# okieraised/rs-face-detection-tflite

Measured on AMD Instinct MI355X. Metric: faces/sec at batch=256 (256x256 back-camera) per GPU, higher is better.
Workload: dtype f32

## Files before the change

rs-face-detection-tflite_amd/csrc/engine.cpp:

```cpp
#include "engine.hpp"
#include "launch.hpp"

#include <mutex>

#include <algorithm>
#include <cstdio>
#include <cstdlib>
#include <cstring>
#include <functional>
#include <stdexcept>

namespace mi {

void hip_check(hipError_t e, const char* what) {
    if (e != hipSuccess) throw std::runtime_error(std::string(what) + ": " + hipGetErrorString(e));
}

namespace {
constexpr int kHeadStreams = 4;

void same_pad(int in, int k, int stride, int out, int* before) {
    int total = std::max(0, (out - 1) * stride + k - in);
    *before = total / 2;
}
// ... 34 lines not shown
}

void Model::invalidate_graphs() {
    if (!graphs_.empty()) (void)hipDeviceSynchronize();
    for (auto& kv : graphs_) hipGraphExecDestroy(kv.second);
    graphs_.clear();
}

void Model::set_option(const std::string& key, int value) {
    if (key == "chunk") chunk_ = std::max(0, value);
    else if (key == "graph") use_graph_ = value != 0;
    else if (key == "fuse") { fuse_level_ = std::min(5, std::max(0, value)); dirty_ = true; }
    else if (key == "res_budget") { res_budget_ = std::min(156, std::max(16, value)) * 1024; dirty_ = true; }
    else if (key == "pipe") { pipe_max_ = std::min(4, std::max(0, value)); dirty_ = true; }
    else if (key == "small_chain") { small_chain_ = std::max(0, std::min(value, 64)); if (d_small_) { hipFree(d_small_); d_small_ = nullptr; small_floats_ = 0; } invalidate_graphs(); }
    else if (key == "pipe_rows") { pipe_rows_ = (value == 1 || value == 2 || value == 4) ? value : 0; }
    else if (key == "pipe_band") { pipe_band_ = std::max(0, std::min(value, 4096)); }
    else if (key == "strip") { strip_ = value != 0; }
    else if (key == "stem_fuse") { stem_fuse_ = value != 0; }
    else if (key == "stem_mfma") { stem_mfma_ = value != 0; }
    else if (key == "pair_fuse") { pair_fuse_ = value != 0; }
    else if (key == "mdb_band") { mdb_band_ = std::max(0, std::min(value, 4096)); }
    else if (key == "mchain") { mchain_ = value != 0; }
    else if (key == "tail") { tail_ = value != 0; dirty_ = true; }
    else if (key == "tail_pre") { tail_pre_ = std::max(0, std::min(value, 2)); }
    else if (key == "tail_g") { tail_g_ = std::max(0, std::min(value, 64)); }
    else if (key == "band") { band_ = std::max(0, std::min(value, 2)); dirty_ = true; }
    else if (key == "band_test_fail") { band_test_fail_ = value != 0; }
    else if (key == "band_test_absent") { band_test_absent_ = std::max(0, std::min(value, 256)); }
    else if (key == "band_test_gen") { band_gen_ = static_cast<unsigned>(std::max(0, value)); band_gen_force_ = true; }
    else if (key == "band_wide") { band_wide_ok_ = value != 0; dirty_ = true; }
    else if (key == "band_fork") { band_fork_ = value != 0; dirty_ = true; }
    else if (key == "band_nw") { band_nw_ = std::max(8, std::min(value, 256)); dirty_ = true; }
    else if (key == "fork") { fork_ = value != 0; }
    else if (key == "heads") { head_streams_opt_ = std::min(kHeadStreams, std::max(1, value)); dirty_ = true; }
    else if (key == "reuse") { reuse_ = value != 0; dirty_ = true; }
    else if (key == "lanes") lanes_ = std::min(4, std::max(1, value));
    else throw std::runtime_error("unknown option '" + key + "'");
    invalidate_graphs();
    chunk_cap_ = 0;
}

int Model::get_option(const std::string& key) const {
    if (key == "chunk") return chunk_;
    if (key == "graph") return use_graph_;
    if (key == "fuse") return fuse_level_;
    if (key == "res_budget") return res_budget_ / 1024;
    if (key == "pipe") return pipe_max_;
    if (key == "small_chain") return small_chain_;
    if (key == "pipe_rows") return pipe_rows_;
    if (key == "pipe_band") return pipe_band_;
    if (key == "strip") return strip_;
    if (key == "stem_fuse") return stem_fuse_;
    if (key == "stem_mfma") return stem_mfma_;
    if (key == "pair_fuse") return pair_fuse_;
    if (key == "mdb_band") return mdb_band_;
    if (key == "mchain") return mchain_;
    if (key == "tail") return tail_;
    if (key == "tail_pre") return tail_pre_;
    if (key == "tail_g") return tail_g_;
    if (key == "band") return band_;
    if (key == "band_fork") return band_fork_;
    if (key == "band_wide") return band_wide_ok_;
    if (key == "band_nw") return band_nw_;
    if (key == "band_fail_streak") return band_fail_streak_;
    if (key == "band_wraps") return band_wraps_;
    if (key == "fork") return fork_;
    if (key == "heads") return head_streams_opt_;
    if (key == "reuse") return reuse_;
    if (key == "lanes") return lanes_;
    throw std::runtime_error("unknown option '" + key + "'");
}

void Model::rebuild() {
    if (d_small_) { hipFree(d_small_); d_small_ = nullptr; small_floats_ = 0; }
    hip_check(hipSetDevice(device_), "hipSetDevice");
    invalidate_graphs();
    plan_ = build_plan(parse_tflite(blob_.data(), blob_.size()), fuse_level_, pipe_max_, res_budget_, tail_ != 0);
    const Graph& g = plan_.graph;
    if (!reuse_) {
// ... 1366 lines not shown
    return stats;
}

void Model::enqueue_chunk(const float* in, int chunk_start, int F, hipStream_t s, std::vector<hipEvent_t>* marks,
                          std::vector<std::string>* labels) {
    const Graph& g = plan_.graph;
    auto mark = [&] {
        if (!marks) return;
        hipEvent_t ev;
        hip_check(hipEventCreate(&ev), "hipEventCreate");
        hip_check(hipEventRecord(ev, s), "hipEventRecord");
        marks->push_back(ev);
    };
    mark();
    const bool fork = fork_ && !marks && lanes_ == 1;
    hipStream_t const trunk = s;
    unsigned used_heads = 0;
    auto node_event = [&](size_t k) {
        if (head_events_.size() < plan_.nodes.size() + 2 + kHeadStreams) head_events_.resize(plan_.nodes.size() + 2 + kHeadStreams, nullptr);
        if (!head_events_[k]) hip_check(hipEventCreateWithFlags(&head_events_[k], hipEventDisableTiming), "hipEventCreate");
        return head_events_[k];
    };
    int fused_behind = 0;
    const bool band = band_use_ && chunk_start == 0;
    for (size_t i = 0; i < plan_.nodes.size(); i++) {
        const Node& n = plan_.nodes[i];
        if (n.kind == Node::Reshape || n.kind == Node::Concat) continue;
        if (band && static_cast<int>(i) >= band_first_ && !band_node_runs_[i]) {
            if (static_cast<int>(i) > band_first_) {
                if (labels) labels->push_back("(inside the band launch)");
                mark();
                continue;
            }
            if (labels) labels->push_back("bandnet_kernel");
            BandLaunch a;
            a.prog = d_band_prog_; a.nstages = band_nstages_; a.NW = band_nw_used_; a.F = F; a.lds_bytes = band_lds_bytes_;
            a.tiles_floats = band_tiles_floats_;
            a.dw_floats = band_dw_floats_; a.ws_frame_floats = band_ws_frame_floats_;
            long fs = 0;
            a.base[0] = d_band_ws_;
            a.base[1] = const_cast<float*>(tensor_ptr(band_stem_out_, in, chunk_start, &fs));
            a.cv2 = band_cv2_ ? 1 : 0;
            a.xb = band_xb_ ? 1 : 0;
            a.wide = band_wide_ ? 1 : 0;
            for (size_t k = 0; k < band_ext_.size(); k++) {
                long efs = 0;
                a.base[2 + k] = band_ext_[k].out_k >= 0 ? d_out_[static_cast<size_t>(band_ext_[k].out_k)] : tensor_ptr_mut(band_ext_[k].tensor, chunk_start, &efs);
            }
            a.consts = d_band_consts_; a.sync = d_band_sync_; a.fail = d_band_fail_;
            a.absent_mod = band_test_absent_;
            int rc = 0;
            for (int rep_ = 0; rep_ < (marks ? profile_inner_ : 1) && rc == 0; rep_++) rc = launch_bandnet(a, trunk);
            if (rc != 0) throw std::runtime_error(std::string("kernel launch failed: ") + hipGetErrorString(static_cast<hipError_t>(rc)));
            for (size_t j = i; fork && j < plan_.nodes.size(); j++)
                if (!band_node_runs_[j] && event_after_[j]) hip_check(record_event(node_event(j), trunk), "hipEventRecord");
            mark();
            continue;
        }
        if (fused_behind > 0) {
            fused_behind--;
            if (labels) labels->push_back("(fused into previous launch)");
            if (fork && event_after_[i]) hip_check(record_event(node_event(i), trunk), "hipEventRecord");
            mark();
            continue;
        }
        s = trunk;
        const bool in_line = band && n.gemm_head && head_wait_[i] >= 0 && !band_node_runs_[static_cast<size_t>(head_wait_[i])];
        if (fork && head_slot_[i] >= 0 && !in_line) {
            while (static_cast<int>(head_streams_.size()) <= head_slot_[i]) {
                hipStream_t st;
                hip_check(hipStreamCreateWithFlags(&st, hipStreamNonBlocking), "hipStreamCreate");
                head_streams_.push_back(st);
            }
            s = head_streams_[head_slot_[i]];
            if (head_wait_[i] >= 0) {
                hip_check(wait_event(s, node_event(static_cast<size_t>(head_wait_[i]))), "hipStreamWaitEvent");
            } else {
                hip_check(record_event(node_event(plan_.nodes.size()), trunk), "hipEventRecord");
                hip_check(wait_event(s, node_event(plan_.nodes.size())), "hipStreamWaitEvent");
            }
            used_heads |= 1u << head_slot_[i];
        }
        const auto& si = g.tensors[n.in[0]].shape;
// ... 31 lines not shown
                    break;
                }
                if (strip_ && stem_fuse_ && node_stem_[i] >= 0 && !u8_.frames) {
                    const size_t j = i + 1;
                    if (node_mwalk_[j] >= 0 && !event_after_[i] && head_slot_[j] < 0) {
                        const Node& c = plan_.nodes[j];
                        const auto& co = g.tensors[c.out].shape;
                        DblockArgs d;
                        long ofs = 0;
                        d.out = tensor_ptr_mut(c.out, chunk_start, &ofs); d.out_fs = ofs;
                        d.B = F; d.H = so[1]; d.W = so[2]; d.C = so[3]; d.Cm = g.tensors[c.members[0].out].shape[3]; d.Co = co[3];
                        d.hi1 = c.members[0].act == ACT_RELU6 ? 6.f : INFINITY;
                        d.hi2 = c.members[1].act == ACT_RELU6 ? 6.f : INFINITY;
                        d.skip1 = 1; d.skip2_from_a = 1;
                        d.act1 = c.members[0].act; d.act2 = c.members[1].act;
                        d.mconsts = d_weights_ + node_mwalk_[j];
                        d.stem_in = ip; d.stem_in_fs = in_fs; d.stem_consts = d_weights_ + node_stem_[i];
                        d.stem_hi = n.act == ACT_RELU6 ? 6.f : INFINITY;
                        d.band_rows = mdb_band_;
                        if (mdblock_kernel_supports(d)) {
                            if (labels) labels->back() = "mdblock_kernel<stem+pair>";
                            rc = launch_mdblock(d, s);
                            fused_behind = 1;
                            break;
                        }
                    }
                }
                ConvArgs a;
                a.in = ip; a.out = op; a.in_fs = in_fs; a.out_fs = out_fs;
                a.w = d_weights_ + node_w_[i];
                a.B = F; a.H = si[1]; a.W = si[2]; a.C = si[3]; a.Ho = so[1]; a.Wo = so[2]; a.Co = so[3]; a.Cop = (a.Co + 3) & ~3;
                a.KH = n.KH; a.KW = n.KW; a.sh = n.sh; a.sw = n.sw;
                if (n.padding == Padding::Same) { same_pad(a.H, a.KH, a.sh, a.Ho, &a.pt); same_pad(a.W, a.KW, a.sw, a.Wo, &a.pl); }
                if (n.ept >= 0) { a.pt = n.ept; a.pl = n.epl; }
                a.ep = ep;
                a.no_mfma = stem_mfma_ ? 0 : 1;
                if (u8_.frames && plan_.storage[n.in[0]].root == plan_.storage[g.inputs[0]].root) {
                    if (!conv_takes_u8(a)) throw std::runtime_error("plan: this graph's first convolution has no u8 input form");
                    a.in_u8 = u8_.frames + static_cast<long>(chunk_start) * u8_.frame_bytes;
                    a.u8_lut = u8_.lut; a.u8_frame_bytes = u8_.frame_bytes; a.u8_row_bytes = u8_.row_bytes;
                }
                if (labels) labels->back() = conv_kernel_label(a);
                rc = launch_conv(a, s);
                break;
            }
            case Node::Dw: {
// ... 258 lines not shown
                if (a.has_dw && n.ept >= 0) { a.pt = n.ept; a.pl = n.epl; }
                a.ep = ep;
                a.w_strip = node_strip_[i] >= 0 ? d_weights_ + node_strip_[i] : nullptr;
                a.w_mwalk = node_mwalk_[i] >= 0 ? d_weights_ + node_mwalk_[i] : nullptr;
                if (strip_ && pair_fuse_ && node_pair_[i] >= 0 && i + 1 < plan_.nodes.size() && !event_after_[i] && head_slot_[i + 1] < 0 && head_slot_[i] < 0) {
                    const Node& nb = plan_.nodes[i + 1];
                    {
                        DblockArgs d;
                        long ofs = 0;
                        d.in = ip; d.in_fs = in_fs;
                        d.out = tensor_ptr_mut(nb.out, chunk_start, &ofs); d.out_fs = ofs;
                        d.B = F; d.H = si[1]; d.W = si[2]; d.C = si[3]; d.Cm = si[3]; d.Co = si[3];
                        d.hi1 = n.act == ACT_RELU6 ? 6.f : INFINITY;
                        d.hi2 = nb.act == ACT_RELU6 ? 6.f : INFINITY;
                        d.skip1 = 1; d.skip2_from_a = 1;
                        d.act1 = n.act; d.act2 = nb.act;
                        d.mconsts = d_weights_ + node_pair_[i];
                        d.band_rows = mdb_band_;
                        const bool apart = d.out + d.out_fs * F <= d.in || d.in + d.in_fs * F <= d.out;
                        if (apart && mdblock_kernel_supports(d)) {
                            if (labels) labels->back() = "mdblock_kernel<pair>";
                            rc = launch_mdblock(d, s);
                            fused_behind = 1;
                            break;
                        }
                    }
                }
                if (strip_ && ms2_kernel_supports(a)) {
                    if (labels) { char buf[96]; labels->back() = ms2_kernel_label(a, buf, sizeof buf); }
                    rc = launch_ms2(a, s);
                    break;
                }
                if (strip_ && mwalk_kernel_supports(a)) {
                    if (labels) { char buf[96]; labels->back() = mwalk_kernel_label(a, buf, sizeof buf); }
                    rc = launch_mwalk(a, s);
                    break;
                }
                const bool strip = strip_ && strip_kernel_supports(a);
                const bool mstrip = strip_ && !strip && mstrip_kernel_supports(a);
                if (mstrip && mchain_ && lanes_ == 1) {
                    std::vector<BlockArgs> run{a};
                    for (size_t j = i + 1; j < plan_.nodes.size() && run.size() < 8; j++) {
                        const Node& m = plan_.nodes[j];
                        if (m.kind != Node::Block || m.w < 0 || m.in.size() != 1 || m.in[0] != plan_.nodes[j - 1].out || node_strip_[j] < 0 || head_slot_[j] >= 0) break;
                        const auto& mi_ = g.tensors[m.in[0]].shape;
                        const auto& mo_ = g.tensors[m.out].shape;
// ... 3 lines not shown
                        bb.out = tensor_ptr_mut(m.out, chunk_start, &bb.out_fs);
                        bb.has_dw = 1;
                        bb.w_dw = d_weights_ + node_w_[j];
                        bb.b_dw = node_b_[j] >= 0 ? d_weights_ + node_b_[j] : nullptr;
                        bb.w_pw = d_weights_ + node_w2_[j];
                        bb.w_strip = d_weights_ + node_strip_[j];
                        bb.B = F; bb.H = mi_[1]; bb.W = mi_[2]; bb.C = mi_[3]; bb.Ho = mo_[1]; bb.Wo = mo_[2]; bb.Co = mo_[3];
                        bb.sh = m.sh; bb.sw = m.sw;
                        if (m.padding == Padding::Same) { same_pad(bb.H, 3, bb.sh, bb.Ho, &bb.pt); same_pad(bb.W, 3, bb.sw, bb.Wo, &bb.pl); }
                        if (m.ept >= 0) break;
                        bb.ep.bias = node_b2_[j] >= 0 ? d_weights_ + node_b2_[j] : nullptr;
                        bb.ep.alpha = node_alpha_[j] >= 0 ? d_weights_ + node_alpha_[j] : nullptr;
                        bb.ep.act = m.act;
                        if (m.res >= 0) {
                            if (m.res != m.in[0] || m.res_mode != RES_DIRECT || m.res_after) break;
                            bb.ep.res = bb.in; bb.ep.res_fs = bb.in_fs; bb.ep.res_mode = RES_DIRECT; bb.ep.res_C = bb.C;
                            bb.ep.res_H = bb.H; bb.ep.res_W = bb.W;
                        }
                        run.push_back(bb);
                        if (!mstrip_chain_supports(run.data(), static_cast<int>(run.size()))) { run.pop_back(); break; }
                    }
                    if (run.size() >= 2) {
                        if (labels) { char buf[96]; snprintf(buf, sizeof buf, "mstrip_chain_kernel<%d,%d>", a.C / 4, a.ep.act == ACT_RELU ? 1 : 0); labels->back() = buf; }
                        rc = launch_mstrip_chain(run.data(), static_cast<int>(run.size()), s);
                        fused_behind = static_cast<int>(run.size()) - 1;
                        break;
                    }
                }
                if (labels) { char buf[96]; labels->back() = strip ? strip_kernel_label(a, buf, sizeof buf) : (mstrip ? mstrip_kernel_label(a, buf, sizeof buf) : block_kernel_label(a, buf, sizeof buf)); }
                rc = strip ? launch_strip(a, s) : (mstrip ? launch_mstrip(a, s) : launch_block(a, s));
                break;
            }
            default: {
                EltArgs a;
                a.a = ip; a.a_fs = in_fs; a.out = op; a.out_fs = out_fs; a.alpha = ep.alpha; a.act = n.act;
                a.B = F; a.H = dim(si, 1); a.W = dim(si, 2); a.C = si.back();
                a.Ho = dim(so, 1); a.Wo = dim(so, 2); a.Co = so.back();
                if (si.size() != 4) { a.H = 1; a.W = 1; a.C = static_cast<int>(g.tensors[n.in[0]].elems()); a.Ho = a.Wo = 1; a.Co = a.C; }
                if (n.kind == Node::Add) {
                    a.b = tensor_ptr(n.in[1], in, chunk_start, &a.b_fs);
                    rc = launch_add(a, s);
                } else if (n.kind == Node::Act) {
                    rc = launch_act(a, s);
                } else if (n.kind == Node::MaxPool) {
                    a.p0 = n.filter_h; a.p1 = n.filter_w; a.p2 = n.sh; a.p3 = n.sw;
                    rc = launch_maxpool(a, s);
                } else if (n.kind == Node::Pad) {
                    const auto& pv = g.tensors[n.pads].i32;
// ... 221 lines not shown
            d_in_stage_ = nullptr;
            hip_check(hipMalloc(reinterpret_cast<void**>(&d_in_stage_), need * sizeof(float)), "hipMalloc stage");
            in_stage_floats_ = need;
        }
        hip_check(hipMemcpyAsync(d_in_stage_, in, need * sizeof(float), hipMemcpyHostToDevice, s), "H2D input");
        din = d_in_stage_;
    }
    run_device(din, batch, s);
    for (int k = 0; k < num_outputs(); k++) {
        if (!outs[k]) continue;
        hip_check(hipMemcpyAsync(outs[k], d_out_[k], output_elems(k) * sizeof(float) * batch,
                                 mem == 0 ? hipMemcpyDeviceToHost : hipMemcpyDeviceToDevice, s), "copy outputs");
    }
    if (mem == 0 || !stream) hip_check(hipStreamSynchronize(s), "hipStreamSynchronize");
}

size_t Model::debug_tensor(int tensor, int frame, float* dst, size_t cap) {
    const Graph& g = plan_.graph;
    if (tensor < 0 || tensor >= static_cast<int>(g.tensors.size())) throw std::runtime_error("tensor index out of range");
    if (frame < 0 || frame >= last_chunk_frames_) throw std::runtime_error("frame outside the last chunk");
    const Storage& st = plan_.storage[tensor];
    bool produced = false;
    for (const Node& n : plan_.nodes) produced |= (n.out == tensor);
    if (!produced) throw std::runtime_error("tensor was fused away (or is an input/constant)");
    long fs;
    float* p = tensor_ptr_mut(tensor, 0, &fs);
    size_t n = std::min(cap, g.tensors[tensor].elems());
    hip_check(hipDeviceSynchronize(), "sync");
    hip_check(hipMemcpy(dst, p + static_cast<long>(frame) * fs, n * sizeof(float), hipMemcpyDeviceToHost), "D2H debug");
    (void)st;
    return n;
}

}
```

rs-face-detection-tflite_amd/csrc/engine.hpp:

```cpp
#pragma once

#include <hip/hip_runtime.h>

#include <map>
#include <memory>
#include <string>
#include <vector>

#include "plan.hpp"

namespace mi {

void hip_check(hipError_t e, const char* what);

class Model {
   public:
    Model(const uint8_t* bytes, size_t n, int device);
    ~Model();
    Model(const Model&) = delete;
    Model& operator=(const Model&) = delete;

    int device() const { return device_; }
    const Graph& graph() const { return plan_.graph; }
    const Plan& plan() const { return plan_; }
// ... 47 lines not shown
    std::vector<hipEvent_t> lane_events_;
    std::vector<int> head_slot_;
    std::vector<int> head_wait_;
    std::vector<char> event_after_;
    std::vector<hipStream_t> head_streams_;
    std::vector<hipEvent_t> head_events_;
    bool dirty_ = true;

    float* d_weights_ = nullptr;
    std::vector<long> node_w_, node_b_, node_w2_, node_b2_, node_alpha_;
    std::vector<long> node_pair_;
    std::vector<long> node_stem_;
    std::vector<long> node_mwalk_;
    std::vector<long> node_strip_;
    struct MemberOff { long w = -1, b = -1, w2 = -1, b2 = -1, alpha = -1, strip = -1; };
    int profile_inner_ = 1;
    std::vector<std::vector<MemberOff>> chain_off_;
    std::vector<std::vector<MemberOff>> chain_head_off_;

    ResStage* d_programs_ = nullptr;
    TailStage* d_tail_programs_ = nullptr;
    std::vector<std::vector<long>> tail_wa_, tail_wc_;
    int mchain_ = 1;
    int tail_ = 1;
    int tail_pre_ = 0;
    int tail_g_ = 0;
    std::vector<std::vector<long>> res_wblk_;
    std::vector<std::vector<long>> res_cblob_;
    std::vector<long> node_prog_;
    float* d_arena_ = nullptr;
    size_t arena_floats_ = 0;
    int chunk_cap_ = 0;
    int batch_cap_ = 0;
    std::vector<float*> d_out_;
    float* d_in_stage_ = nullptr;
    size_t in_stage_floats_ = 0;
    int last_chunk_frames_ = 0;

    int band_ = 1;
    int band_nw_ = 128;
    int band_nw_used_ = 0;
    bool band_ready_ = false;
    bool band_use_ = false;
    bool band_ran_ = false;
    bool band_test_fail_ = false;
    int band_test_absent_ = 0;
    int band_fail_streak_ = 0;
    bool band_disabled_ = false;
    unsigned band_gen_ = 0;
    bool band_gen_force_ = false;
    int band_wraps_ = 0;
    size_t band_ws_bytes_ = 0;
    int band_first_ = 0;
    int band_stem_out_ = -1;
    int band_nstages_ = 0, band_lds_bytes_ = 0, band_max_frames_ = 0, band_dw_floats_ = 0;
    int band_tiles_floats_ = 0;
    long band_ws_frame_floats_ = 0;
    struct BandExt { int out_k = -1, tensor = -1; };
    std::vector<BandExt> band_ext_;
    std::vector<char> band_node_runs_;
// ... 38 lines not shown
```

rs-face-detection-tflite_amd/csrc/kernels.hpp:

```cpp
#pragma once

#include <cstddef>
#include <cstdint>

namespace mi {

enum ActKind : int { ACT_NONE = 0, ACT_RELU = 1, ACT_RELU6 = 2, ACT_PRELU = 3 };
enum ResMode : int { RES_NONE = 0, RES_DIRECT = 1, RES_MAXPOOL = 2, RES_UP2X = 3 };

struct Epilogue {
    const float* bias = nullptr;
    const float* alpha = nullptr;
    const float* res = nullptr;
    long res_fs = 0;
    int res_mode = RES_NONE;
    int res_C = 0;
    int res_W = 0, res_H = 0;
    int act = ACT_NONE;
    int res_after = 0;
};

struct ConvArgs {
    const float* in = nullptr;
    const uint8_t* in_u8 = nullptr;
// ... 238 lines not shown
bool strip_shape_ok(int C, int Co);
int strip_consts_floats(int C);
void strip_pack_consts(int C, const float* w_dw, const float* b_dw, const float* w_pw, const float* bias, const float* alpha, int act, float* dst);
const char* strip_kernel_label(const BlockArgs& a, char* buf, size_t cap);
int launch_mwalk(const BlockArgs& a, void* stream);
bool mwalk_kernel_supports(const BlockArgs& a);
bool mwalk_shape_ok(int W, int C, int Co);
int mwalk_consts_floats(int W, int C, int Co);
void mwalk_pack_consts(int W, int C, int Co, const float* w_dw, const float* b_dw, const float* w_pw, const float* bias, const float* alpha, int act, float* dst);
const char* mwalk_kernel_label(const BlockArgs& a, char* buf, size_t cap);
int launch_ms2(const BlockArgs& a, void* stream);
bool ms2_kernel_supports(const BlockArgs& a);
bool ms2_shape_ok(int W, int C, int Co, bool skip);
int ms2_consts_floats(int W, int C, int Co, bool skip);
void ms2_pack_consts(int W, int C, int Co, bool skip, const float* w_dw, const float* b_dw, const float* w_pw, const float* bias, const float* alpha, int act, float* dst);
const char* ms2_kernel_label(const BlockArgs& a, char* buf, size_t cap);
int launch_mstrip(const BlockArgs& a, void* stream);
bool mstrip_kernel_supports(const BlockArgs& a);
bool mstrip_shape_ok(int C, int Co);
int mstrip_consts_floats(int C);
void mstrip_pack_consts(int C, const float* w_dw, const float* b_dw, const float* w_pw, const float* bias, const float* alpha, int act, float* dst);
const char* mstrip_kernel_label(const BlockArgs& a, char* buf, size_t cap);
bool mstrip_chain_supports(const BlockArgs* blocks, int n);
int launch_mstrip_chain(const BlockArgs* blocks, int n, void* stream);
bool strip_pipe_supports(const BlockArgs* blocks, int n);
bool strip_pipe_shape_ok(int C, int W);
bool strip_tail_shape_ok(int C, int Co, int H, int W);
int strip_consts_s2_floats(int C, int Co);
void strip_pack_consts_s2(int C, int Co, const float* w_dw, const float* b_dw, const float* w_pw, const float* bias, const float* alpha, int act, float* dst);
int launch_strip_pipe(const BlockArgs* blocks, int n, void* stream);
const char* strip_pipe_label(const BlockArgs* blocks, int n, char* buf, size_t cap);
int strip_pipe_rows_per_step(int H, int hint = 0);
int launch_chain(const ChainArgs& a, void* stream);

struct BneckBlock {
    const float* w1 = nullptr;
    const float* w2 = nullptr;
    const float* consts = nullptr;
    float hi1 = 0.f, hi2 = 0.f;
    const float* mconsts = nullptr;
    int act1 = ACT_RELU, act2 = ACT_RELU;
};
constexpr int kMaxBneck = 6;
struct BneckArgs {
    const float* in = nullptr;
    float* out = nullptr;
    long in_fs = 0, out_fs = 0;
// ... 154 lines not shown
```

rs-face-detection-tflite_amd/csrc/mstrip_kernels.hip:

```cpp
#include <hip/hip_runtime.h>

#include <algorithm>
#include <cstdint>
#include <cstdio>
#include <cstdlib>
#include <type_traits>
#include <utility>

#include "kernels.hpp"
#include "launch.hpp"

namespace mi {

namespace {

typedef float v2f __attribute__((ext_vector_type(2)));
typedef float f32x4 __attribute__((ext_vector_type(4)));

struct MstripArgs {
    const float* in;
    float* out;
    const float* consts;
    long in_fs, out_fs;
    int B, H;
    int bands, band_rows;
    int has_res;
    float hi;
    unsigned long long* stamps;
};

constexpr int kMstripChain = 8;
struct MstripChainArgs {
    const float* in[kMstripChain];
    float* out[kMstripChain];
    const float* consts[kMstripChain];
    long in_fs[kMstripChain], out_fs[kMstripChain];
    int has_res[kMstripChain];
    float hi[kMstripChain];
    int nblocks, B, H;
};

template <int CK>
struct MK {
    static constexpr int C = 4 * CK, MT = C / 16;
    static constexpr int QP = CK + 1;
    static constexpr int PS = 4 * QP;
    static constexpr int IMG_F = 34 * PS;
    static constexpr int DPX = 64 / QP;
    static constexpr int NLD = 32 / DPX;
    static_assert(32 % DPX == 0 && NLD == 8, "eight DMA instructions per row (two source bases, four immediate offsets each)");
    static_assert((16 * PS) % 64 == 0 && 16 * PS / 64 < 256, "ds_read2st64_b32 reaches the second pixel tile");
    static constexpr int OFF_A = 0, A_F = CK * MT * 64, OFF_TAP = A_F, TAP_F = CK * 48, OFF_BIAS = OFF_TAP + TAP_F, OFF_SLOPE = OFF_BIAS + C, TOTAL = OFF_SLOPE + C;
    static constexpr int WG_F = A_F + 2 * C + TAP_F;
    static constexpr int NBUF = 2;
};

template <int N>
__device__ __forceinline__ void mwait_vm() { __builtin_amdgcn_s_waitcnt((N & 15) | ((N >> 4) << 14) | 0x0F70); }
__device__ __forceinline__ void mwave_sync() {
    __builtin_amdgcn_fence(__ATOMIC_RELEASE, "wavefront");
    __builtin_amdgcn_wave_barrier();
    __builtin_amdgcn_fence(__ATOMIC_ACQUIRE, "wavefront");
}

template <class F, int... KS>
__device__ __forceinline__ void mfor_each(F&& f, std::integer_sequence<int, KS...>) { (f(std::integral_constant<int, KS>{}), ...); }

template <int CK, bool RELU>
__global__ __launch_bounds__(256, 2) void mstrip_kernel(MstripArgs a) {
    using K = MK<CK>;
    constexpr int C = K::C, MT = K::MT, PS = K::PS, QP = K::QP, IMG_F = K::IMG_F, NLD = K::NLD, NBUF = K::NBUF;
    extern __shared__ __attribute__((aligned(16))) float lds[];
#ifdef MI_MSTRIP_STAMPS
    unsigned long long st_acc[7] = {0, 0, 0, 0, 0, 0, 0}, st_prev = __builtin_amdgcn_s_memtime();
#define MI_MSTAMP(k) { __builtin_amdgcn_sched_barrier(0); unsigned long long t_ = __builtin_amdgcn_s_memtime(); asm volatile("s_waitcnt lgkmcnt(0)" ::: "memory"); st_acc[k] += t_ - st_prev; st_prev = t_; __builtin_amdgcn_sched_barrier(0); }
#else
#define MI_MSTAMP(k)
// ... 484 lines not shown
    };
    step(std::false_type{}, y0 - 1, accA, accB);
    step(std::false_type{}, y0, accB, accA);
    for (int r = y0 + 1; r <= y1; r += 2) {
        step(std::true_type{}, r, accA, accB);
        if (r + 1 > y1) break;
        step(std::true_type{}, r + 1, accB, accA);
    }
    asm volatile("s_waitcnt vmcnt(0)" ::: "memory");
    if (more) {
        float* nx = lds + ((blk + 1) & 1) * K::WG_F;
#pragma unroll
        for (int k = 0; k < NPRE; k++) {
            const int i = threadIdx.x + 512 * k;
            if (i < K::WG_F / 4) reinterpret_cast<float4*>(nx)[i] = pre[k];
        }
    }
    asm volatile("s_waitcnt vmcnt(0) lgkmcnt(0)" ::: "memory");
    __builtin_amdgcn_s_barrier();
    asm volatile("" ::: "memory");
  }
}

}

bool mstrip_shape_ok(int C, int Co) {
    static const bool off = getenv("MI_NO_MSTRIP") != nullptr;
    return !off && C == Co && C == 48;
}

bool mstrip_kernel_supports(const BlockArgs& a) {
    if (!a.w_strip || !a.has_dw || a.sh != 1 || a.sw != 1 || a.pt != 1 || a.pl != 1) return false;
    if (!mstrip_shape_ok(a.C, a.Co) || a.W != 32 || a.H != a.Ho || a.W != a.Wo || a.H < 2) return false;
    if (a.ep.res_mode != RES_NONE) {
        if (a.ep.res_after) return false;
        if (a.ep.res_mode != RES_DIRECT || a.ep.res != a.in || a.ep.res_fs != a.in_fs || a.ep.res_C != a.C) return false;
    }
    static const int min_b = getenv("MI_MSTRIP_MIN_B") ? atoi(getenv("MI_MSTRIP_MIN_B")) : 32;
    if (a.B < min_b) return false;
    auto aligned16 = [](const void* p) { return (reinterpret_cast<uintptr_t>(p) & 15) == 0; };
    return aligned16(a.in) && aligned16(a.out) && !(a.in_fs & 3) && !(a.out_fs & 3);
}

int mstrip_consts_floats(int C) { return C == 48 ? MK<12>::TOTAL : 0; }

void mstrip_pack_consts(int C, const float* w_dw, const float* b_dw, const float* w_pw, const float* bias, const float* alpha, int act, float* dst) {
    using K = MK<12>;
    std::fill(dst, dst + mstrip_consts_floats(C), 0.f);
    for (int ks = 0; ks < K::C / 4; ks++)
        for (int mt = 0; mt < K::MT; mt++)
            for (int l = 0; l < 64; l++) dst[K::OFF_A + (ks * K::MT + mt) * 64 + l] = w_pw[(size_t)(16 * mt + (l & 15)) * C + 4 * ks + (l >> 4)];
    for (int ks = 0; ks < K::C / 4; ks++)
        for (int kq = 0; kq < 4; kq++)
            for (int t = 0; t < 9; t++) dst[K::OFF_TAP + (ks * 4 + kq) * 12 + t] = w_dw[t * C + 4 * ks + kq];
    for (int c = 0; c < C; c++) {
        double acc = bias ? bias[c] : 0.0;
        if (b_dw)
            for (int k = 0; k < C; k++) acc += (double)w_pw[(size_t)c * C + k] * b_dw[k];
        dst[K::OFF_BIAS + c] = (float)acc;
        dst[K::OFF_SLOPE + c] = act == ACT_PRELU ? alpha[c] : (act == ACT_NONE ? 1.f : 0.f);
    }
}

const char* mstrip_kernel_label(const BlockArgs& a, char* buf, size_t cap) {
    snprintf(buf, cap, "mstrip_kernel<%d,%d>", a.C / 4, a.ep.act == ACT_RELU ? 1 : 0);
    return buf;
}

bool mstrip_chain_supports(const BlockArgs* blocks, int n) {
    static const bool off = getenv("MI_NO_MSTRIP_CHAIN") != nullptr;
    if (off || n < 2 || n > kMstripChain) return false;
    for (int k = 0; k < n; k++) {
        const BlockArgs& a = blocks[k];
        if (!mstrip_kernel_supports(a) || a.H != 32 || a.B != blocks[0].B || (a.ep.act == ACT_RELU) != (blocks[0].ep.act == ACT_RELU)) return false;
        if (k && a.in != blocks[k - 1].out) return false;
    }
    return true;
}

int launch_mstrip_chain(const BlockArgs* blocks, int n, void* stream) {
    using K = MK<12>;
    if (!mstrip_chain_supports(blocks, n)) return (int)hipErrorInvalidValue;
    MstripChainArgs ca{};
    ca.nblocks = n; ca.B = blocks[0].B; ca.H = blocks[0].H;
    for (int k = 0; k < n; k++) {
        const BlockArgs& a = blocks[k];
        ca.in[k] = a.in; ca.out[k] = a.out; ca.consts[k] = a.w_strip; ca.in_fs[k] = a.in_fs; ca.out_fs[k] = a.out_fs;
        ca.has_res[k] = a.ep.res_mode == RES_DIRECT;
        ca.hi[k] = a.ep.act == ACT_RELU6 ? 6.f : INFINITY;
    }
    const size_t lds_bytes = (size_t)(2 * K::WG_F + 8 * K::NBUF * K::IMG_F) * 4;
    const dim3 grid((unsigned)ca.B);
    hipStream_t s = (hipStream_t)stream;
    if (blocks[0].ep.act == ACT_RELU) {
        auto kern = mstrip_chain_kernel<12, true>;
        if (hipError_t e = allow_full_lds(reinterpret_cast<const void*>(kern)); e != hipSuccess) return (int)e;
        return (int)launch_kernel(kern, grid, dim3(512), lds_bytes, s, ca);
    }
    auto kern = mstrip_chain_kernel<12, false>;
    if (hipError_t e = allow_full_lds(reinterpret_cast<const void*>(kern)); e != hipSuccess) return (int)e;
    return (int)launch_kernel(kern, grid, dim3(512), lds_bytes, s, ca);
}

unsigned long long* g_mstrip_stamps = nullptr;

int launch_mstrip(const BlockArgs& a, void* stream) {
    using K = MK<12>;
    MstripArgs ma;
    ma.stamps = g_mstrip_stamps;
    ma.in = a.in; ma.out = a.out; ma.consts = a.w_strip; ma.in_fs = a.in_fs; ma.out_fs = a.out_fs;
    ma.B = a.B; ma.H = a.H;
    static const int forced = getenv("MI_MSTRIP_BAND") ? atoi(getenv("MI_MSTRIP_BAND")) : 0;
    long bands = std::max<long>(1, (8L * device_cu_count() + a.B / 2) / std::max(1, a.B));
    int rows = (int)((a.H + bands - 1) / bands);
    rows = std::max(rows, std::min(a.H, 4));
    if (forced > 0) rows = std::min(forced, a.H);
    ma.band_rows = rows;
    ma.bands = (a.H + rows - 1) / rows;
    ma.has_res = a.ep.res_mode == RES_DIRECT;
    ma.hi = a.ep.act == ACT_RELU6 ? 6.f : INFINITY;
    hipStream_t s = (hipStream_t)stream;
    const long units = (long)a.B * ma.bands;
    const size_t lds_bytes = (size_t)(K::WG_F + 4 * K::NBUF * K::IMG_F) * 4;
    const dim3 grid((unsigned)((units + 3) / 4));
    if (a.ep.act == ACT_RELU) {
        auto kern = mstrip_kernel<12, true>;
        if (hipError_t e = allow_full_lds(reinterpret_cast<const void*>(kern)); e != hipSuccess) return (int)e;
// ... 9 lines not shown
```

Baseline: 214,900.

## Add wavefront-pipelined mstrip chain kernel with one wave per block

Adds a new mstrip_pipe_kernel in which each wave owns one depthwise+pointwise block of the chain and passes rows to the next wave through double-buffered LDS, so intermediate activations never go to global memory. Rows stream from global memory into LDS via direct-to-LDS loads issued by the first wave, and the waves advance in a staggered row pipeline synchronised by barriers. It is on by default through a new 'mpipe' option, and the engine now tracks which intermediate tensors are no longer written so debug reads of them fail. The trade-offs are fewer threads per workgroup (64*n), many barriers, and a pipeline fill and drain phase at the start and end of each image.

Result: no change. 215,800 (median of 6 runs) (+0.4%).

```diff
diff --git a/rs-face-detection-tflite_amd/csrc/engine.cpp b/rs-face-detection-tflite_amd/csrc/engine.cpp
--- a/rs-face-detection-tflite_amd/csrc/engine.cpp
+++ b/rs-face-detection-tflite_amd/csrc/engine.cpp
@@ -80,6 +80,7 @@
     else if (key == "pair_fuse") { pair_fuse_ = value != 0; }
     else if (key == "mdb_band") { mdb_band_ = std::max(0, std::min(value, 4096)); }
     else if (key == "mchain") { mchain_ = value != 0; }
+    else if (key == "mpipe") { mpipe_ = value != 0; }
     else if (key == "tail") { tail_ = value != 0; dirty_ = true; }
     else if (key == "tail_pre") { tail_pre_ = std::max(0, std::min(value, 2)); }
     else if (key == "tail_g") { tail_g_ = std::max(0, std::min(value, 64)); }
@@ -114,6 +115,7 @@
     if (key == "pair_fuse") return pair_fuse_;
     if (key == "mdb_band") return mdb_band_;
     if (key == "mchain") return mchain_;
+    if (key == "mpipe") return mpipe_;
     if (key == "tail") return tail_;
     if (key == "tail_pre") return tail_pre_;
     if (key == "tail_g") return tail_g_;
@@ -1526,6 +1528,8 @@
         return head_events_[k];
     };
     int fused_behind = 0;
+    bool fused_writes = false;
+    unwritten_.assign(g.tensors.size(), 0);
     const bool band = band_use_ && chunk_start == 0;
     for (size_t i = 0; i < plan_.nodes.size(); i++) {
         const Node& n = plan_.nodes[i];
@@ -1563,6 +1567,7 @@
         }
         if (fused_behind > 0) {
             fused_behind--;
+            if (!fused_writes) unwritten_[static_cast<size_t>(plan_.nodes[i - 1].out)] = 1;
             if (labels) labels->push_back("(fused into previous launch)");
             if (fork && event_after_[i]) hip_check(record_event(node_event(i), trunk), "hipEventRecord");
             mark();
@@ -1640,6 +1645,7 @@
                             if (labels) labels->back() = "mdblock_kernel<stem+pair>";
                             rc = launch_mdblock(d, s);
                             fused_behind = 1;
+                            fused_writes = false;
                             break;
                         }
                     }
@@ -1944,6 +1950,7 @@
                             if (labels) labels->back() = "mdblock_kernel<pair>";
                             rc = launch_mdblock(d, s);
                             fused_behind = 1;
+                            fused_writes = false;
                             break;
                         }
                     }
@@ -1993,8 +2000,10 @@
                     }
                     if (run.size() >= 2) {
                         if (labels) { char buf[96]; snprintf(buf, sizeof buf, "mstrip_chain_kernel<%d,%d>", a.C / 4, a.ep.act == ACT_RELU ? 1 : 0); labels->back() = buf; }
-                        rc = launch_mstrip_chain(run.data(), static_cast<int>(run.size()), s);
+                        const bool pipe = mpipe_ && mstrip_pipe_supports(run.data(), static_cast<int>(run.size()));
+                        rc = launch_mstrip_chain(run.data(), static_cast<int>(run.size()), s, pipe);
                         fused_behind = static_cast<int>(run.size()) - 1;
+                        fused_writes = !pipe;
                         break;
                     }
                 }
@@ -2262,7 +2271,8 @@
     const Storage& st = plan_.storage[tensor];
     bool produced = false;
     for (const Node& n : plan_.nodes) produced |= (n.out == tensor);
-    if (!produced) throw std::runtime_error("tensor was fused away (or is an input/constant)");
+    if (!produced || (static_cast<size_t>(tensor) < unwritten_.size() && unwritten_[static_cast<size_t>(tensor)]))
+        throw std::runtime_error("tensor was fused away (or is an input/constant)");
     long fs;
     float* p = tensor_ptr_mut(tensor, 0, &fs);
     size_t n = std::min(cap, g.tensors[tensor].elems());
diff --git a/rs-face-detection-tflite_amd/csrc/engine.hpp b/rs-face-detection-tflite_amd/csrc/engine.hpp
--- a/rs-face-detection-tflite_amd/csrc/engine.hpp
+++ b/rs-face-detection-tflite_amd/csrc/engine.hpp
@@ -93,6 +93,7 @@
     TailStage* d_tail_programs_ = nullptr;
     std::vector<std::vector<long>> tail_wa_, tail_wc_;
     int mchain_ = 1;
+    int mpipe_ = 1;
     int tail_ = 1;
     int tail_pre_ = 0;
     int tail_g_ = 0;
@@ -107,6 +108,7 @@
     float* d_in_stage_ = nullptr;
     size_t in_stage_floats_ = 0;
     int last_chunk_frames_ = 0;
+    std::vector<char> unwritten_;
 
     int band_ = 1;
     int band_nw_ = 128;
diff --git a/rs-face-detection-tflite_amd/csrc/kernels.hpp b/rs-face-detection-tflite_amd/csrc/kernels.hpp
--- a/rs-face-detection-tflite_amd/csrc/kernels.hpp
+++ b/rs-face-detection-tflite_amd/csrc/kernels.hpp
@@ -284,7 +284,8 @@
 void mstrip_pack_consts(int C, const float* w_dw, const float* b_dw, const float* w_pw, const float* bias, const float* alpha, int act, float* dst);
 const char* mstrip_kernel_label(const BlockArgs& a, char* buf, size_t cap);
 bool mstrip_chain_supports(const BlockArgs* blocks, int n);
-int launch_mstrip_chain(const BlockArgs* blocks, int n, void* stream);
+bool mstrip_pipe_supports(const BlockArgs* blocks, int n);
+int launch_mstrip_chain(const BlockArgs* blocks, int n, void* stream, bool pipe);
 bool strip_pipe_supports(const BlockArgs* blocks, int n);
 bool strip_pipe_shape_ok(int C, int W);
 bool strip_tail_shape_ok(int C, int Co, int H, int W);
diff --git a/rs-face-detection-tflite_amd/csrc/mstrip_kernels.hip b/rs-face-detection-tflite_amd/csrc/mstrip_kernels.hip
--- a/rs-face-detection-tflite_amd/csrc/mstrip_kernels.hip
+++ b/rs-face-detection-tflite_amd/csrc/mstrip_kernels.hip
@@ -38,6 +38,17 @@
     int has_res[kMstripChain];
     float hi[kMstripChain];
     int nblocks, B, H;
+};
+
+struct MpipeArgs {
+    const float* in;
+    float* out;
+    const float* consts[kMstripChain];
+    long in_fs, out_fs;
+    int has_res[kMstripChain];
+    float hi[kMstripChain];
+    int nblocks;
+    unsigned long long* stamps;
 };
 
 template <int CK>
@@ -53,6 +64,9 @@
     static constexpr int OFF_A = 0, A_F = CK * MT * 64, OFF_TAP = A_F, TAP_F = CK * 48, OFF_BIAS = OFF_TAP + TAP_F, OFF_SLOPE = OFF_BIAS + C, TOTAL = OFF_SLOPE + C;
     static constexpr int WG_F = A_F + 2 * C + TAP_F;
     static constexpr int NBUF = 2;
+    static constexpr int PIPE_CA_F = A_F + 2 * C;
+    static constexpr int PIPE_IMG_S = 33 * PS;
+    static constexpr size_t pipe_lds_bytes(int n) { return (size_t)(n * PIPE_CA_F + (2 * n * 33 + 1) * PS) * 4; }
 };
 
 template <int N>
@@ -583,6 +597,264 @@
   }
 }
 
+template <int CK, bool RELU>
+__global__ __launch_bounds__(512, 2) void mstrip_pipe_kernel(MpipeArgs pa) {
+    using K = MK<CK>;
+    constexpr int C = K::C, MT = K::MT, PS = K::PS, QP = K::QP, IMG_S = K::PIPE_IMG_S, NLD = K::NLD, H = 32;
+    extern __shared__ __attribute__((aligned(16))) float lds[];
+#ifdef MI_MSTRIP_STAMPS
+    unsigned long long st_acc[7] = {0, 0, 0, 0, 0, 0, 0}, st_prev = __builtin_amdgcn_s_memtime();
+    const unsigned long long st_t0 = st_prev;
+#define MI_PSTAMP(k) { __builtin_amdgcn_sched_barrier(0); unsigned long long t_ = __builtin_amdgcn_s_memtime(); asm volatile("s_waitcnt lgkmcnt(0)" ::: "memory"); st_acc[k] += t_ - st_prev; st_prev = t_; __builtin_amdgcn_sched_barrier(0); }
+#else
+#define MI_PSTAMP(k)
+#endif
+    (void)NLD;
+    const int lane = threadIdx.x & 63;
+    const int wave = __builtin_amdgcn_readfirstlane(threadIdx.x >> 6);
+    const int kq = lane >> 4, p = lane & 15;
+    const int n = pa.nblocks, b = blockIdx.x;
+    const bool first = wave == 0, last = wave == n - 1;
+    float* const wgc = lds + wave * K::PIPE_CA_F;
+    float* const img = lds + n * K::PIPE_CA_F + 2 * wave * IMG_S;
+    float* const nimg = img + 2 * IMG_S;
+    const float* const cs = pa.consts[wave];
+    const int has_res = pa.has_res[wave];
+    const float hi = pa.hi[wave];
+    const float* const in = pa.in + (long)b * pa.in_fs;
+
+    const int goff = ((lane / QP) * C + 4 * min(lane % QP, CK - 1)) * 4;
+    const unsigned lds_img = __builtin_amdgcn_readfirstlane((unsigned)(uintptr_t)(__attribute__((address_space(3))) float*)img);
+    auto issue_row = [&](int r, int bi) {
+        const char* src = reinterpret_cast<const char*>(in + (long)r * 32 * C);
+        const char* src1 = src + (NLD / 2) * K::DPX * C * 4;
+        const unsigned dstb = lds_img + (unsigned)((bi * IMG_S + PS) * 4);
+        constexpr int ACTIVE = K::DPX * QP;
+        static_assert(ACTIVE > 32 && ACTIVE < 64, "exec mask written as two 32-bit halves");
+        unsigned long long saved;
+#define MI_MS_DMA(base, k) "s_add_u32 m0, m0, %7\n\ts_nop 0\n\tglobal_load_lds_dwordx4 %3, " base " offset:" #k "*%8\n\t"
+        asm volatile("s_mov_b64 %0, exec\n\ts_mov_b32 exec_lo, -1\n\ts_mov_b32 exec_hi, %6\n\t"
+                     "s_mov_b32 m0, %4\n\ts_nop 0\n\tglobal_load_lds_dwordx4 %3, %1\n\t"
+                     MI_MS_DMA("%1", 1) MI_MS_DMA("%1", 2) MI_MS_DMA("%1", 3)
+                     "s_add_u32 m0, m0, %5\n\ts_nop 0\n\tglobal_load_lds_dwordx4 %3, %2\n\t"
+                     MI_MS_DMA("%2", 1) MI_MS_DMA("%2", 2) MI_MS_DMA("%2", 3)
+                     "s_mov_b64 exec, %0"
+                     : "=&s"(saved)
+                     : "s"(src), "s"(src1), "v"(goff), "s"(dstb), "n"((NLD / 2) * K::DPX * PS * 4 - (NLD / 2 - 1) * K::DPX * (PS - C) * 4),
+                       "n"((1u << (ACTIVE - 32)) - 1), "n"(K::DPX * (PS - C) * 4), "n"(K::DPX * C * 4)
+                     : "memory", "scc", "m0");
+#undef MI_MS_DMA
+    };
+    auto fix_row = [&](int r, int bi) {
+        if (r >= 0 && r < H) return;
+        float zz = 0.f;
+        asm volatile("" : "+v"(zz));
+        const float4 z = make_float4(zz, zz, zz, zz);
+        float* part = img + bi * IMG_S + PS;
+        constexpr int N4 = 32 * QP;
+#pragma unroll
+        for (int k = 0; k < (N4 + 63) / 64; k++)
+            if (64 * (k + 1) <= N4 || lane < N4 - 64 * k) *reinterpret_cast<float4*>(part + 4 * (lane + 64 * k)) = z;
+    };
+    if (lane < 2 * QP) {
+        const int col = lane / QP, qd = lane - col * QP;
+#pragma unroll
+        for (int bi = 0; bi < 2; bi++) *reinterpret_cast<float4*>(img + bi * IMG_S + col * 33 * PS + 4 * qd) = make_float4(0.f, 0.f, 0.f, 0.f);
+    }
+    if (first) issue_row(0, 1);
+    {
+        static_assert(K::A_F % 256 == 0 && 2 * C <= 256, "whole float4 per lane");
+        f32x4 cv[K::A_F / 256 + 1];
+#pragma unroll
+        for (int k = 0; k < K::A_F / 256; k++) cv[k] = reinterpret_cast<const f32x4*>(cs + K::OFF_A)[lane + 64 * k];
+        if (lane < 2 * C / 4) cv[K::A_F / 256] = reinterpret_cast<const f32x4*>(cs + K::OFF_BIAS)[lane];
+#pragma unroll
+        for (int k = 0; k < K::A_F / 256; k++) reinterpret_cast<f32x4*>(wgc)[lane + 64 * k] = cv[k];
+        if (lane < 2 * C / 4) reinterpret_cast<f32x4*>(wgc + K::A_F)[lane] = cv[K::A_F / 256];
+    }
+    float tap[CK][9];
+    {
+        const float4* tp = reinterpret_cast<const float4*>(cs + K::OFF_TAP) + kq * 3;
+#pragma unroll
+        for (int ks = 0; ks < CK; ks++) {
+            const float4 t0 = tp[ks * 12], t1 = tp[ks * 12 + 1], t2 = tp[ks * 12 + 2];
+            tap[ks][0] = t0.x; tap[ks][1] = t0.y; tap[ks][2] = t0.z; tap[ks][3] = t0.w;
+            tap[ks][4] = t1.x; tap[ks][5] = t1.y; tap[ks][6] = t1.z; tap[ks][7] = t1.w;
+            tap[ks][8] = t2.x;
+        }
+#pragma unroll
+        for (int ks = 0; ks < CK; ks++)
+#pragma unroll
+            for (int t = 0; t < 9; t++) asm volatile("" : "+v"(tap[ks][t]));
+    }
+    auto step_sync = [&] {
+        asm volatile("s_waitcnt lgkmcnt(0)" ::: "memory");
+        __builtin_amdgcn_s_barrier();
+        asm volatile("" ::: "memory");
+    };
+    step_sync();
+    MI_PSTAMP(0)
+    for (int s = 0; s < 2 * wave; s++) step_sync();
+    MI_PSTAMP(1)
+
+    const float* xme = img + p * PS + kq;
+    const float* sme = img + (1 + p) * PS + 4 * kq;
+    const float* ame = wgc + lane;
+    const unsigned ooff = (unsigned)(p * C + 4 * kq) * 4u;
+    float* const nme = nimg + (1 + p) * PS + 4 * kq;
+
+    float accA[CK][2], accB[CK][2];
+    f32x4 D[MT][2];
+#pragma unroll
+    for (int ks = 0; ks < CK; ks++) accA[ks][0] = accA[ks][1] = accB[ks][0] = accB[ks][1] = 0.f;
+
+    auto init_D = [&](int bi) {
+        float4 bs[MT], x[MT][2];
+#pragma unroll
+        for (int mt = 0; mt < MT; mt++) bs[mt] = *reinterpret_cast<const float4*>(wgc + K::A_F + 16 * mt + 4 * kq);
+        if (has_res) {
+#pragma unroll
+            for (int mt = 0; mt < MT; mt++)
+#pragma unroll
+                for (int nt = 0; nt < 2; nt++) x[mt][nt] = *reinterpret_cast<const float4*>(sme + bi * IMG_S + 16 * nt * PS + 16 * mt);
+#pragma unroll
+            for (int mt = 0; mt < MT; mt++)
+#pragma unroll
+                for (int nt = 0; nt < 2; nt++) D[mt][nt] = f32x4{x[mt][nt].x + bs[mt].x, x[mt][nt].y + bs[mt].y, x[mt][nt].z + bs[mt].z, x[mt][nt].w + bs[mt].w};
+        } else {
+#pragma unroll
+            for (int mt = 0; mt < MT; mt++) D[mt][0] = D[mt][1] = f32x4{bs[mt].x, bs[mt].y, bs[mt].z, bs[mt].w};
+        }
+    };
+    typedef __attribute__((address_space(1))) char gchar;
+    typedef __attribute__((address_space(1))) f32x4 gf32x4;
+    auto act = [&](int mt, f32x4 v) {
+        if (RELU) return f32x4{fmaxf(v.x, 0.f), fmaxf(v.y, 0.f), fmaxf(v.z, 0.f), fmaxf(v.w, 0.f)};
+        const float4 sl = *reinterpret_cast<const float4*>(wgc + K::A_F + C + 16 * mt + 4 * kq);
+        return f32x4{fminf(fmaxf(v.x, 0.f) + sl.x * fminf(v.x, 0.f), hi), fminf(fmaxf(v.y, 0.f) + sl.y * fminf(v.y, 0.f), hi),
+                     fminf(fmaxf(v.z, 0.f) + sl.z * fminf(v.z, 0.f), hi), fminf(fmaxf(v.w, 0.f) + sl.w * fminf(v.w, 0.f), hi)};
+    };
+    auto epilogue = [&](int y) {
+        if (last) {
+            gchar* dst = (gchar*)(pa.out + (long)b * pa.out_fs + (long)y * 32 * C);
+            asm volatile("" : "+s"(dst));
+#pragma unroll
+            for (int mt = 0; mt < MT; mt++)
+#pragma unroll
+                for (int nt = 0; nt < 2; nt++) *(gf32x4*)(dst + ooff + (unsigned)((16 * nt * C + 16 * mt) * 4)) = act(mt, D[mt][nt]);
+        } else {
+            float* const ndst = nme + ((y + 1) & 1) * IMG_S;
+#pragma unroll
+            for (int mt = 0; mt < MT; mt++)
+#pragma unroll
+                for (int nt = 0; nt < 2; nt++) *reinterpret_cast<f32x4*>(ndst + 16 * nt * PS + 16 * mt) = act(mt, D[mt][nt]);
+        }
+    };
+
+    const unsigned x_lds = (unsigned)(uintptr_t)(__attribute__((address_space(3))) float*)const_cast<float*>(xme);
+    const unsigned a_lds = (unsigned)(uintptr_t)(__attribute__((address_space(3))) float*)const_cast<float*>(ame);
+    auto row = [&](auto emit, int bi, float (&aPN)[CK][2], float (&aC)[CK][2]) {
+        constexpr bool EMIT = decltype(emit)::value;
+        const unsigned xr = x_lds + (unsigned)(bi * IMG_S * 4), ar = a_lds;
+        float xs[2][3][2], av[2][MT];
+        auto load_ks = [&](auto ksc, float (&x)[3][2], float (&aw)[MT]) {
+            constexpr int ks = decltype(ksc)::value;
+            const unsigned xa = xr, aa = ar;
+#pragma unroll
+            for (int dx = 0; dx < 3; dx++) {
+                asm volatile("ds_read_b32 %0, %1 offset:%2" : "=v"(x[dx][0]) : "v"(xa), "n"((dx * PS + 4 * ks) * 4));
+                asm volatile("ds_read_b32 %0, %1 offset:%2" : "=v"(x[dx][1]) : "v"(xa), "n"((dx * PS + 4 * ks + 16 * PS) * 4));
+            }
+            if constexpr (EMIT) {
+#pragma unroll
+                for (int mt = 0; mt < MT; mt++) asm volatile("ds_read_b32 %0, %1 offset:%2" : "=v"(aw[mt]) : "v"(aa), "n"((ks * MT + mt) * 64 * 4));
+            }
+        };
+        auto landed = [&](float (&x)[3][2], float (&aw)[MT]) {
+#pragma unroll
+            for (int dx = 0; dx < 3; dx++) asm volatile("" : "+v"(x[dx][0]), "+v"(x[dx][1]));
+            if constexpr (EMIT) {
+#pragma unroll
+                for (int mt = 0; mt < MT; mt++) asm volatile("" : "+v"(aw[mt]));
+            }
+        };
+        auto kstep = [&](auto ksc) {
+            constexpr int ks = decltype(ksc)::value;
+            if constexpr (ks + 1 < CK) load_ks(std::integral_constant<int, ks + 1>{}, xs[(ks + 1) & 1], av[(ks + 1) & 1]);
+            float (&x)[3][2] = xs[ks & 1];
+            float (&aw)[MT] = av[ks & 1];
+            const float (&w)[9] = tap[ks];
+            float pch[2];
+#pragma unroll
+            for (int nt = 0; nt < 2; nt++) {
+                float n_ = x[0][nt] * w[0], c = aC[ks][nt], pc = aPN[ks][nt];
+#pragma unroll
+                for (int dx = 0; dx < 3; dx++) {
+                    if (EMIT) pc = __builtin_fmaf(x[dx][nt], w[6 + dx], pc);
+                    if (dx) n_ = __builtin_fmaf(x[dx][nt], w[dx], n_);
+                    c = __builtin_fmaf(x[dx][nt], w[3 + dx], c);
+                }
+                aC[ks][nt] = c;
+                aPN[ks][nt] = n_;
+                asm volatile("" : "+v"(aC[ks][nt]), "+v"(aPN[ks][nt]));
+                pch[nt] = pc;
+            }
+            if constexpr (EMIT) {
+#pragma unroll
+                for (int mt = 0; mt < MT; mt++) {
+                    D[mt][0] = __builtin_amdgcn_mfma_f32_16x16x4f32(aw[mt], pch[0], D[mt][0], 0, 0, 0);
+                    D[mt][1] = __builtin_amdgcn_mfma_f32_16x16x4f32(aw[mt], pch[1], D[mt][1], 0, 0, 0);
+                }
+            }
+            asm volatile("s_waitcnt lgkmcnt(0)" ::: "memory");
+            if constexpr (ks + 1 < CK) landed(xs[(ks + 1) & 1], av[(ks + 1) & 1]);
+            __builtin_amdgcn_sched_barrier(0);
+        };
+        load_ks(std::integral_constant<int, 0>{}, xs[0], av[0]);
+        asm volatile("s_waitcnt lgkmcnt(0)" ::: "memory");
+        landed(xs[0], av[0]);
+        __builtin_amdgcn_sched_barrier(0);
+        mfor_each(kstep, std::make_integer_sequence<int, CK>{});
+    };
+
+    auto step = [&](auto emit, int r, float (&aPN)[CK][2], float (&aC)[CK][2]) {
+        const int bi = (r + 1) & 1;
+        if (first) {
+            if (r >= 0) mwait_vm<0>();
+            if (r + 1 >= 1 && r + 1 < H) issue_row(r + 1, bi ^ 1);
+        }
+        fix_row(r, bi);
+        mwave_sync();
+        MI_PSTAMP(2)
+        row(emit, bi, aPN, aC);
+        __builtin_amdgcn_sched_barrier(0);
+        if constexpr (decltype(emit)::value) epilogue(r - 1);
+        __builtin_amdgcn_sched_barrier(0);
+        init_D(bi);
+        __builtin_amdgcn_sched_barrier(0);
+        MI_PSTAMP(3)
+        step_sync();
+        MI_PSTAMP(4)
+    };
+    step(std::false_type{}, -1, accA, accB);
+    step(std::false_type{}, 0, accB, accA);
+    for (int r = 1; r <= H; r += 2) {
+        step(std::true_type{}, r, accA, accB);
+        step(std::true_type{}, r + 1, accB, accA);
+    }
+    for (int s = 2 * wave; s < 2 * (n - 1); s++) step_sync();
+    MI_PSTAMP(5)
+#ifdef MI_MSTRIP_STAMPS
+    if (pa.stamps && lane == 0) {
+        unsigned long long* o = pa.stamps + ((long)b * kMstripChain + wave) * 8;
+        for (int k = 0; k < 6; k++) o[k] = st_acc[k];
+        o[6] = st_t0;
+        o[7] = st_prev;
+    }
+#endif
+#undef MI_PSTAMP
+}
+
 }
 
 bool mstrip_shape_ok(int C, int Co) {
@@ -628,6 +900,8 @@
     return buf;
 }
 
+unsigned long long* g_mstrip_stamps = nullptr;
+
 bool mstrip_chain_supports(const BlockArgs* blocks, int n) {
     static const bool off = getenv("MI_NO_MSTRIP_CHAIN") != nullptr;
     if (off || n < 2 || n > kMstripChain) return false;
@@ -639,9 +913,44 @@
     return true;
 }
 
-int launch_mstrip_chain(const BlockArgs* blocks, int n, void* stream) {
+bool mstrip_pipe_supports(const BlockArgs* blocks, int n) {
+    if (!mstrip_chain_supports(blocks, n)) return false;
+    const BlockArgs &f = blocks[0], &l = blocks[n - 1];
+    const float* in_end = f.in + f.in_fs * (f.B - 1) + (long)f.H * f.W * f.C;
+    const float* out_end = l.out + l.out_fs * (l.B - 1) + (long)l.H * l.W * l.Co;
+    const bool apart = out_end <= f.in || in_end <= l.out;
+    const bool same = f.in == l.out && f.in_fs == l.out_fs;
+    return (apart || same) && MK<12>::pipe_lds_bytes(n) <= 160 * 1024;
+}
+
+int launch_mstrip_chain(const BlockArgs* blocks, int n, void* stream, bool pipe) {
     using K = MK<12>;
     if (!mstrip_chain_supports(blocks, n)) return (int)hipErrorInvalidValue;
+    if (pipe) {
+        if (!mstrip_pipe_supports(blocks, n)) return (int)hipErrorInvalidValue;
+        MpipeArgs pa{};
+        pa.nblocks = n;
+        pa.in = blocks[0].in; pa.in_fs = blocks[0].in_fs;
+        pa.out = blocks[n - 1].out; pa.out_fs = blocks[n - 1].out_fs;
+        pa.stamps = g_mstrip_stamps;
+        for (int k = 0; k < n; k++) {
+            const BlockArgs& a = blocks[k];
+            pa.consts[k] = a.w_strip;
+            pa.has_res[k] = a.ep.res_mode == RES_DIRECT;
+            pa.hi[k] = a.ep.act == ACT_RELU6 ? 6.f : INFINITY;
+        }
+        const size_t lds_bytes = K::pipe_lds_bytes(n);
+        const dim3 grid((unsigned)blocks[0].B), block((unsigned)(64 * n));
+        hipStream_t s = (hipStream_t)stream;
+        if (blocks[0].ep.act == ACT_RELU) {
+            auto kern = mstrip_pipe_kernel<12, true>;
+            if (hipError_t e = allow_full_lds(reinterpret_cast<const void*>(kern)); e != hipSuccess) return (int)e;
+            return (int)launch_kernel(kern, grid, block, lds_bytes, s, pa);
+        }
+        auto kern = mstrip_pipe_kernel<12, false>;
+        if (hipError_t e = allow_full_lds(reinterpret_cast<const void*>(kern)); e != hipSuccess) return (int)e;
+        return (int)launch_kernel(kern, grid, block, lds_bytes, s, pa);
+    }
     MstripChainArgs ca{};
     ca.nblocks = n; ca.B = blocks[0].B; ca.H = blocks[0].H;
     for (int k = 0; k < n; k++) {
@@ -662,8 +971,6 @@
     if (hipError_t e = allow_full_lds(reinterpret_cast<const void*>(kern)); e != hipSuccess) return (int)e;
     return (int)launch_kernel(kern, grid, dim3(512), lds_bytes, s, ca);
 }
-
-unsigned long long* g_mstrip_stamps = nullptr;
 
 int launch_mstrip(const BlockArgs& a, void* stream) {
     using K = MK<12>;
```
